# lixirui142/VidToMe

Hardware: AMD Instinct MI355X
Metric: denoising steps/sec, 16-frame 512x512 SD-1.5 chunk, ratio=0.5 (higher is better)
Workload: dtype f16 tokens; matching f16-MFMA filter + f32 exact refine (f32-identical indices); attention f16 MFMA with f32 accumulate

## Files before the change

### include/vidtome_hip.h

```cpp
#ifndef VIDTOME_HIP_H
#define VIDTOME_HIP_H

#include <stddef.h>
#include <stdint.h>

#ifdef __cplusplus
extern "C" {
#endif

#define VTM_ABI_VERSION 2

enum vtm_dtype { VTM_F32 = 0, VTM_F16 = 1, VTM_BF16 = 2 };

enum vtm_status {
    VTM_OK = 0,
    VTM_EINVAL = -1,
    VTM_ELAUNCH = -2,
    VTM_EWORKSPACE = -3
};

typedef void *vtm_stream_t;

int vtm_version(void);
const char *vtm_last_error(void);
// ... 128 lines not shown
                                    const int32_t *q_count, void *ws, size_t ws_bytes, vtm_stream_t stream);
size_t vtm_attention_kv_bounded_ws_bytes(int64_t B, int64_t h, int64_t Mq, int64_t Mk, int64_t d);

int vtm_transpose_cols(const void *x, int64_t ldx, int dtype, int64_t BF, int64_t N, int64_t C, void *out, int64_t ldo,
                       vtm_stream_t stream);

size_t vtm_fold_keys_ws_bytes(int64_t B, int64_t M, int64_t n_ids);
int vtm_fold_keys(const int32_t *cur, int64_t B, int64_t M, int64_t L, const int32_t *cid, int64_t Ma, int64_t n_ids,
                  int dtype, void *ws, size_t ws_bytes, int32_t *key_sel, uint32_t *k_bias, int64_t ldkb,
                  int32_t *k_count, vtm_stream_t stream);
int vtm_attention_kv_folded(const void *q, int64_t ldq, const void *k, int64_t ldk, const void *vt, int64_t ldvt,
                            void *out, int64_t ldo, int dtype, int64_t B, int64_t h, int64_t Mq, int64_t Mqp,
                            int64_t Mk, int64_t Mkp, int64_t d, float scale, const int32_t *q_count,
                            const int32_t *k_count, const uint32_t *k_bias, int64_t ldkb, void *ws, size_t ws_bytes,
                            vtm_stream_t stream);

size_t vtm_compact_queries_ws_bytes(int64_t B, int64_t Nd);
int vtm_compact_queries(const int32_t *loc, int64_t B, int64_t Ml, int64_t U, int64_t Nd, void *ws, size_t ws_bytes,
                        int32_t *qc, int32_t *tmap, int32_t *count, vtm_stream_t stream);

int64_t vtm_panel_rows(int64_t n);
int vtm_to_panels(const void *x, int dtype, int64_t rows, int64_t C, const int32_t *order, void *out, int64_t rows_pad,
                  vtm_stream_t stream);
int vtm_layernorm_panels(const void *x, const void *gamma, const void *beta, int dtype, int64_t rows, int64_t C, float eps,
                         void *out, int64_t panel_rows, vtm_stream_t stream);
int vtm_gather_panels(const void *x0, int64_t P0, const void *x1, int64_t P1, int dtype, int64_t B, int64_t C,
                      const int32_t *map, int64_t map_ld, const int32_t *map2, int64_t n, void *out, int64_t rows_per_sample,
                      vtm_stream_t stream);
int vtm_ff_geglu(const void *x_panels, int64_t n, int64_t n_pad, const void *w1_panels, int64_t D, int64_t w_rows_pad,
                 int64_t K, const float *bias, int dtype, void *out_panels, vtm_stream_t stream);
int vtm_linear_panels(const void *x_panels, int64_t n, int64_t n_pad, const void *w_panels, int64_t N, int64_t w_rows_pad,
                      int64_t K, const float *bias, const void *resid, int dtype, void *out, int64_t ldo,
                      vtm_stream_t stream);

int vtm_cfg_ddim(const void *x, const void *eps_uncond, const void *eps_cond, int dtype, int64_t n,
                 float guidance, float a, float b, float c, float d, void *eps_out, void *x_out,
                 vtm_stream_t stream);

int vtm_layernorm(const void *x, const void *gamma, const void *beta, int dtype, int64_t rows, int64_t C,
                  float eps, void *out, vtm_stream_t stream);

int vtm_geglu(const void *x, int dtype, int64_t rows, int64_t D, void *out, vtm_stream_t stream);

int vtm_linear_rows(const void *x0, int64_t P0, const void *x1, int64_t P1, int dtype, int64_t B, int64_t K,
                    const int32_t *rows, int64_t rows_ld, const int32_t *rows2, int64_t n, const void *W,
                    const void *bias, int64_t N, void *out, int64_t ldo, int64_t out_batch_stride,
                    int transposed, vtm_stream_t stream);

enum { VTM_LINEAR_NONE = 0, VTM_LINEAR_RESID = 1, VTM_LINEAR_GEGLU = 2 };
int vtm_linear_f32(const float *x0, int64_t P0, const float *x1, int64_t P1, int64_t B, int64_t K,
                   const int32_t *rows, int64_t rows_ld, const int32_t *rows2, int64_t n, const float *W,
                   const float *bias, int64_t N, int epilogue, const float *resid, void *out, int out_dtype,
                   int64_t ldo, int64_t out_batch_stride, int transposed, vtm_stream_t stream);

int vtm_lora_fold(const void *w, int dtype, const float *up, const float *down, int64_t c_out, int64_t c_in,
                  int64_t r, void *out, vtm_stream_t stream);

int vtm_dora_norms(const void *w, int dtype, const float *up, const float *down, int64_t c_out, int64_t c_in,
                   int64_t r, int64_t k_dora, float *norms, vtm_stream_t stream);
int vtm_dora_fold(const void *w, int dtype, const float *up, const float *down, const float *magnitude,
                  const float *norms, int64_t c_out, int64_t c_in, int64_t r, int64_t k_dora, void *out,
                  vtm_stream_t stream);

int vtm_loha_delta(const float *w1a, const float *w1b, const float *w2a, const float *w2b, int64_t c_out, int64_t c_in,
                   int64_t r, int accumulate, float *delta, vtm_stream_t stream);
int vtm_lokr_delta(const float *w1, const float *w2, int64_t a1, int64_t b1, int64_t a2, int64_t b2, int64_t c_out,
// ... 9 lines not shown
```

### vidtome_amd/_lib.py

```python
from __future__ import annotations

import ctypes
import functools
import os
import threading
from typing import Optional, Tuple

import torch

_HERE = os.path.dirname(os.path.abspath(__file__))
ABI_VERSION = 2
LIB_PATH = os.environ.get("VIDTOME_HIP_LIB") or os.path.join(_HERE, "lib", "libvidtome_hip.so")

VTM_F32, VTM_F16, VTM_BF16 = 0, 1, 2
ROW_PAD, K_PAD = 256, 32

_DT = {torch.float32: VTM_F32, torch.float16: VTM_F16, torch.bfloat16: VTM_BF16}

_vp, _i64, _int, _f32 = ctypes.c_void_p, ctypes.c_int64, ctypes.c_int, ctypes.c_float
_lib: Optional[ctypes.CDLL] = None

_SIGNATURES = {
    "vtm_version": ([], _int),
    "vtm_last_error": ([], ctypes.c_char_p),
# ... 29 lines not shown
    "vtm_unmerge_add": ([_vp, _i64, _vp, _vp, _int, _i64, _i64, _i64, _vp, _vp], _int),
    "vtm_merge_reduce": ([_vp, _int, _i64, _i64, _i64, _vp, _vp, _vp, _vp, _i64, _i64, _int, _vp, _i64, _i64, _vp], _int),
    "vtm_attention": ([_vp, _i64, _vp, _i64, _vp, _i64, _vp, _i64, _int, _i64, _i64, _i64, _i64, _i64, _f32,
                       _int, _vp, ctypes.c_size_t, _vp], _int),
    "vtm_attention_ws_bytes": ([_i64, _i64, _i64, _i64, _i64], ctypes.c_size_t),
    "vtm_attention_kv": ([_vp, _i64, _vp, _i64, _vp, _i64, _vp, _i64, _int, _i64, _i64, _i64, _i64, _i64, _i64, _i64,
                          _f32, _int, _vp, ctypes.c_size_t, _vp], _int),
    "vtm_attention_kv_sets": ([_vp, _i64, _vp, _i64, _vp, _i64, _vp, _i64, _int, _i64, _i64, _i64, _i64, _i64, _i64, _f32,
                               _int, ctypes.POINTER(_i64), ctypes.POINTER(_i64), ctypes.POINTER(_f32), _vp], _int),
    "vtm_attention_kv_sets_masked": ([_vp, _i64, _vp, _i64, _vp, _i64, _vp, _i64, _int, _i64, _i64, _i64, _i64, _i64, _i64, _f32,
                                      _int, ctypes.POINTER(_i64), ctypes.POINTER(_i64), ctypes.POINTER(_f32),
                                      ctypes.POINTER(_int), _vp, _i64, _i64, _vp], _int),
    "vtm_attention_kv_bias": ([_vp, _i64, _vp, _i64, _vp, _i64, _vp, _i64, _int, _i64, _i64, _i64, _i64, _i64, _i64, _i64,
                               _f32, _vp, _i64, _i64, _vp], _int),
    "vtm_attention_kv_bounded": ([_vp, _i64, _vp, _i64, _vp, _i64, _vp, _i64, _int, _i64, _i64, _i64, _i64, _i64, _i64, _i64,
                                  _f32, _vp, _vp, ctypes.c_size_t, _vp], _int),
    "vtm_attention_kv_shared_bounded": ([_vp, _i64, _vp, _i64, _vp, _i64, _vp, _i64, _int, _i64, _i64, _i64, _i64, _i64, _i64, _i64,
                                         _f32, _int, _vp, _vp, ctypes.c_size_t, _vp], _int),
    "vtm_attention_kv_bounded_ws_bytes": ([_i64, _i64, _i64, _i64, _i64], ctypes.c_size_t),
    "vtm_anchor_maps": ([_vp, _i64, _i64, _vp, _i64, _i64, _i64, _i64, _i64, _vp, _i64, _vp, _vp, _vp, _vp], _int),
    "vtm_transpose_cols": ([_vp, _i64, _int, _i64, _i64, _i64, _vp, _i64, _vp], _int),
    "vtm_fold_keys_ws_bytes": ([_i64, _i64, _i64], ctypes.c_size_t),
    "vtm_fold_keys": ([_vp, _i64, _i64, _i64, _vp, _i64, _i64, _int, _vp, ctypes.c_size_t, _vp, _vp, _i64, _vp, _vp], _int),
    "vtm_attention_kv_folded": ([_vp, _i64, _vp, _i64, _vp, _i64, _vp, _i64, _int, _i64, _i64, _i64, _i64, _i64, _i64, _i64,
                                 _f32, _vp, _vp, _vp, _i64, _vp, ctypes.c_size_t, _vp], _int),
    "vtm_compact_queries_ws_bytes": ([_i64, _i64], ctypes.c_size_t),
    "vtm_compact_queries": ([_vp, _i64, _i64, _i64, _i64, _vp, ctypes.c_size_t, _vp, _vp, _vp, _vp], _int),
    "vtm_panel_rows": ([_i64], _i64),
    "vtm_to_panels": ([_vp, _int, _i64, _i64, _vp, _vp, _i64, _vp], _int),
    "vtm_layernorm_panels": ([_vp, _vp, _vp, _int, _i64, _i64, _f32, _vp, _i64, _vp], _int),
    "vtm_gather_panels": ([_vp, _i64, _vp, _i64, _int, _i64, _i64, _vp, _i64, _vp, _i64, _vp, _i64, _vp], _int),
    "vtm_ff_geglu": ([_vp, _i64, _i64, _vp, _i64, _i64, _i64, _vp, _int, _vp, _vp], _int),
    "vtm_linear_panels": ([_vp, _i64, _i64, _vp, _i64, _i64, _i64, _vp, _vp, _int, _vp, _i64, _vp], _int),
    "vtm_cfg_ddim": ([_vp, _vp, _vp, _int, _i64, _f32, _f32, _f32, _f32, _f32, _vp, _vp, _vp], _int),
    "vtm_layernorm": ([_vp, _vp, _vp, _int, _i64, _i64, _f32, _vp, _vp], _int),
    "vtm_geglu": ([_vp, _int, _i64, _i64, _vp, _vp], _int),
    "vtm_linear_rows": ([_vp, _i64, _vp, _i64, _int, _i64, _i64, _vp, _i64, _vp, _i64, _vp, _vp, _i64, _vp, _i64, _i64,
                         _int, _vp], _int),
    "vtm_lora_fold": ([_vp, _int, _vp, _vp, _i64, _i64, _i64, _vp, _vp], _int),
    "vtm_dora_norms": ([_vp, _int, _vp, _vp, _i64, _i64, _i64, _i64, _vp, _vp], _int),
    "vtm_dora_fold": ([_vp, _int, _vp, _vp, _vp, _vp, _i64, _i64, _i64, _i64, _vp, _vp], _int),
    "vtm_loha_delta": ([_vp, _vp, _vp, _vp, _i64, _i64, _i64, _int, _vp, _vp], _int),
    "vtm_lokr_delta": ([_vp, _vp, _i64, _i64, _i64, _i64, _i64, _i64, _int, _vp, _vp], _int),
    "vtm_delta_fold": ([_vp, _int, _vp, _i64, _i64, _vp, _vp], _int),
    "vtm_linear_f32": ([_vp, _i64, _vp, _i64, _i64, _i64, _vp, _i64, _vp, _i64, _vp, _vp, _i64, _int, _vp, _vp, _int, _i64,
                        _i64, _int, _vp], _int),
}


def exported_symbols():
    return sorted(_SIGNATURES)


def lib() -> ctypes.CDLL:
    global _lib
    if _lib is None:
        if not os.path.exists(LIB_PATH):
            raise RuntimeError(
                f"{LIB_PATH} is missing: build it with `python -m vidtome_amd.build` (hipcc, gfx950). "
                "vidtome_amd has no CPU / eager fallback.")
        L = ctypes.CDLL(LIB_PATH)
        for name, (argtypes, restype) in _SIGNATURES.items():
            fn = getattr(L, name)
            fn.argtypes = argtypes
            fn.restype = restype
        if L.vtm_version() != ABI_VERSION:
# ... 719 lines not shown
    return out


@_on_device
def ff_geglu(x_panels: torch.Tensor, n: int, w1_panels: torch.Tensor, D: int, bias: Optional[torch.Tensor]) -> torch.Tensor:
    K = x_panels.shape[0] * 8
    out = torch.empty((D // 8, x_panels.shape[1], 8), dtype=x_panels.dtype, device=x_panels.device)
    _check(lib().vtm_ff_geglu(_ptr(x_panels), n, x_panels.shape[1], _ptr(w1_panels), D, w1_panels.shape[1], K, _ptr(bias),
                              dtype_code(x_panels), _ptr(out), _stream()), "vtm_ff_geglu")
    return out


@_on_device
def linear_panels(x_panels: torch.Tensor, n: int, w_panels: torch.Tensor, N: int, bias: Optional[torch.Tensor],
                  resid: Optional[torch.Tensor] = None, out: Optional[torch.Tensor] = None) -> torch.Tensor:
    K = x_panels.shape[0] * 8
    if x_panels.stride(2) != 1 or x_panels.stride(1) != 8 or w_panels.stride(2) != 1 or w_panels.stride(1) != 8 \
            or w_panels.shape[0] * 8 != K:
        raise RuntimeError("linear_panels: operands must be (K / 8, rows, 8) panel tensors (or row ranges of one)")
    if out is None:
        out = torch.empty((n, N), dtype=x_panels.dtype, device=x_panels.device)
    if out.stride(1) != 1 or out.shape[0] < n or out.shape[1] < N:
        raise RuntimeError("linear_panels: out must be an (n, N) view, contiguous along its rows")
    if resid is not None:
        _req(resid, "resid")
        if resid.numel() != n * N or resid.dtype != out.dtype or out.stride(0) != N:
            raise RuntimeError("linear_panels: residual shape / dtype mismatch")
    _check(lib().vtm_linear_panels(_ptr(x_panels), n, x_panels.stride(0) // 8, _ptr(w_panels), N, w_panels.stride(0) // 8, K,
                                   _ptr(bias), _ptr(resid), dtype_code(x_panels), out.data_ptr(), out.stride(0), _stream()),
           "vtm_linear_panels")
    return out


@_on_device
def gather_panels(x0: torch.Tensor, x1: Optional[torch.Tensor], rows: Optional[torch.Tensor], rows2: Optional[torch.Tensor],
                  n: int) -> torch.Tensor:
    _req(x0, "x0")
    B, P0, C = x0.shape
    P1 = 0 if x1 is None else _req(x1, "x1").shape[1]
    n_pad = panel_rows(n)
    out = torch.empty((C // 8, B * n_pad, 8), dtype=x0.dtype, device=x0.device)
    _check(lib().vtm_gather_panels(_ptr(x0), P0, _ptr(x1), P1, dtype_code(x0), B, C, _ptr(rows),
                                   0 if rows is None else rows.shape[1], _ptr(rows2), n, _ptr(out), n_pad, _stream()),
           "vtm_gather_panels")
    return out


@_on_device
def lora_fold(w: torch.Tensor, up: torch.Tensor, down: torch.Tensor, out: Optional[torch.Tensor] = None) -> torch.Tensor:
    _req(w, "w"), _req(up, "up"), _req(down, "down")
    c_out, c_in = w.shape
    r = up.shape[1]
    if up.dtype != torch.float32 or down.dtype != torch.float32 or tuple(up.shape) != (c_out, r) \
            or tuple(down.shape) != (r, c_in) or up.device != w.device or down.device != w.device:
        raise RuntimeError("lora_fold: up must be (c_out, r) and down (r, c_in) fp32 tensors on w's device")
    if out is None:
        out = torch.empty_like(w)
    _check(lib().vtm_lora_fold(_ptr(w), dtype_code(w), _ptr(up), _ptr(down), c_out, c_in, r, _ptr(_req(out, "out")),
                               _stream()), "vtm_lora_fold")
    return out


def _fold_operands(what: str, w: torch.Tensor, up: torch.Tensor, down: torch.Tensor, k_dora: int) -> Tuple[int, int, int]:
    _req(w, "w"), _req(up, "up"), _req(down, "down")
    c_out, c_in = w.shape
    r = up.shape[1]
# ... 96 lines not shown
```

### vidtome_amd/csrc/ff.hip

```cpp
#include "common.h"

#include <algorithm>
#include <cstdlib>
#include <type_traits>

namespace {

constexpr int FBD = 128;
constexpr int FBS = 256;
constexpr int FBK = 64;
constexpr int THREADS = 256;
constexpr int MAX_TILES_PER_WG = 16;

typedef float f32x16 __attribute__((ext_vector_type(16)));
typedef _Float16 h16x8 __attribute__((ext_vector_type(8)));
typedef __bf16 b16x8 __attribute__((ext_vector_type(8)));
typedef uint32_t u32x4 __attribute__((ext_vector_type(4)));
typedef __attribute__((address_space(3))) void lds_void;

template <typename T> struct Mma;
template <> struct Mma<__half> {
    __device__ static f32x16 run(u32x4 a, u32x4 b, f32x16 c) {
        return __builtin_amdgcn_mfma_f32_32x32x16_f16(__builtin_bit_cast(h16x8, a), __builtin_bit_cast(h16x8, b), c, 0, 0, 0);
    }
    __device__ static uint16_t bits(float v) { return __half_as_ushort(__float2half_rn(v)); }
    __device__ static float round(float v) { return __half2float(__float2half_rn(v)); }
};
template <> struct Mma<vtm_bf16> {
    __device__ static f32x16 run(u32x4 a, u32x4 b, f32x16 c) {
        return __builtin_amdgcn_mfma_f32_32x32x16_bf16(__builtin_bit_cast(b16x8, a), __builtin_bit_cast(b16x8, b), c, 0, 0, 0);
    }
    __device__ static uint16_t bits(float v) { return __bfloat16_as_ushort(__float2bfloat16(v)); }
    __device__ static float round(float v) { return __bfloat162float(__float2bfloat16(v)); }
};

__device__ __forceinline__ float gelu_erf(float g) {
    const float x = __builtin_fabsf(g) * 0.70710678118654752440f;
    const float t = __builtin_amdgcn_rcpf(__builtin_fmaf(0.3275911f, x, 1.0f));
    float p = __builtin_fmaf(1.061405429f, t, -1.453152027f);
    p = __builtin_fmaf(p, t, 1.421413741f);
    p = __builtin_fmaf(p, t, -0.284496736f);
    p = __builtin_fmaf(p, t, 0.254829592f);
    const float e = p * t * __builtin_amdgcn_exp2f(-x * x * 1.4426950408889634f);
    return 0.5f * g * (g < 0.0f ? e : 2.0f - e);
}

enum { EPI_GEGLU = 0, EPI_ROWS = 1 };

struct Epi {
    const float *bias;
    void *out;
    int64_t out_rows_pad;
    int64_t ldo;
    const void *resid;
    int64_t n;
    int64_t N;
    int64_t nbias;
};

template <typename T, int EPI>
__global__ __launch_bounds__(THREADS, 2) void panel_gemm_kernel(
    const uint4 *__restrict__ ah, const uint4 *__restrict__ bh, int64_t Ns_pad, int64_t Nd_pad, int64_t C_pad,
    int ns_tiles, int nd_tiles, int nsplit, int tiles_per_split, int total_src_tiles, int patch_tiles, Epi E) {
    __shared__ __attribute__((aligned(16))) uint4 sA[2][8 * FBD];
    __shared__ float sBias[MAX_TILES_PER_WG * FBD];
    __shared__ __attribute__((aligned(16))) uint16_t sOut[EPI == EPI_ROWS ? 4 * 32 * (FBD + 8) : 8];

    const int tid = threadIdx.x, lane = tid & 63;
    const int wave = __builtin_amdgcn_readfirstlane(tid >> 6);
    const int l31 = lane & 31, kh = lane >> 5;

    const int xcd = blockIdx.x & 7, slot = blockIdx.x >> 3;
    const int per_group = patch_tiles * nsplit;
    const int grp = (slot / per_group) * 8 + xcd;
    const int q = slot % per_group;
    const int stg = grp * patch_tiles + q % patch_tiles;
    const int split = q / patch_tiles;
    if (stg >= total_src_tiles) return;
    const int st_ = stg % ns_tiles;
    const int jt0 = split * tiles_per_split;
    const int jt1 = min(jt0 + tiles_per_split, nd_tiles);
    if (jt0 >= jt1) return;

    const int KT = (int)(C_pad / FBK);
    const int steps = (jt1 - jt0) * KT;
    const uint4 *srch = ah, *dsth = bh;
    const int64_t srow0 = (int64_t)st_ * FBS + wave * 64;

    __shared__ Epi sE;
    if (tid == 0) sE = E;
    {
        const int cnt = (jt1 - jt0) * FBD;
        const float *bsrc = E.bias != nullptr ? E.bias + (int64_t)jt0 * FBD : nullptr;
#pragma unroll
        for (int k = 0; k < MAX_TILES_PER_WG * FBD / THREADS; ++k) {
            const int i = tid + k * THREADS;
            if (i < cnt) sBias[i] = (bsrc != nullptr && (int64_t)jt0 * FBD + i < E.nbias) ? bsrc[i] : 0.0f;
        }
    }

    constexpr int NB = 2, PG = 2;
    const uint32_t voff_b = (uint32_t)(kh * Ns_pad + srow0 + l31) * 16u;
    const int64_t bgroup = 2 * Ns_pad;
    u32x4 rb[4][2];
    auto await_b = [&](auto count_tag, u32x4 (&r)[2]) {
// ... 147 lines not shown
                    if constexpr (s < 3) fn[j] = __builtin_bit_cast(u32x4, sA[buf][((s + 1) * 2 + kh) * FBD + j * 32 + l31]);
                    else fn[j] = __builtin_bit_cast(u32x4, sA[buf ^ 1][kh * FBD + j * 32 + l31]);
                } else if (j < 6) {
                    if constexpr (s < 2) load_b1(pb, s + 2, j - 4, rb[s + 2][j - 4]);
                    else load_b1(pbn, s - 2, j - 4, rb[s - 2][j - 4]);
                } else {
                    if constexpr (s == 0) load_a_piece(pa1, buf ^ 1, j - 4);
                    if constexpr (s == 3) load_a_piece(pa2, buf, j - 6);
                    if constexpr (s == 1)
                        asm volatile("global_load_dword %0, %1, %2" : "=v"(am[j - 6]) : "v"(voff_m), "s"(dummy_rows));
                }
                __builtin_amdgcn_sched_barrier(0);
            }
        };
        await_b(std::integral_constant<int, NB + PG>{}, rb[0]);
        if (kt == 0) group(std::integral_constant<int, 0>{}, std::true_type{});
        else group(std::integral_constant<int, 0>{}, std::false_type{});
        group(std::integral_constant<int, 1>{}, std::false_type{});
        group(std::integral_constant<int, 2>{}, std::false_type{});
        asm volatile("s_waitcnt vmcnt(%0) lgkmcnt(0)" ::"n"(2 * NB + 2) : "memory");
        __syncthreads();
        group(std::integral_constant<int, 3>{}, std::false_type{});
        if (wrap) {
            epilogue(jt);
            ++jt;
        }
        kt = kt1;
        pb = pbn;
        pa1 = pa2;
    }
    asm volatile("s_waitcnt vmcnt(0)" ::: "memory");
}

template <typename T>
__global__ __launch_bounds__(256) void to_panels_kernel(const T *__restrict__ x, int64_t rows, int64_t C, int64_t rows_pad,
                                                        const int32_t *__restrict__ order, uint4 *__restrict__ out) {
    const int64_t G = C / 8;
    const int64_t i = (int64_t)blockIdx.x * blockDim.x + threadIdx.x;
    if (i >= rows_pad * G) return;
    const int64_t g = i % G, r = i / G;
    uint4 v = make_uint4(0, 0, 0, 0);
    if (r < rows) {
        const int64_t src = order ? order[r] : r;
        if (src >= 0) v = *reinterpret_cast<const uint4 *>(x + src * C + g * 8);
    }
    out[g * rows_pad + r] = v;
}

template <typename T>
__global__ __launch_bounds__(256) void gather_panels_kernel(const T *__restrict__ x0, int64_t P0, const T *__restrict__ x1,
                                                            int64_t P1, int64_t B, int64_t C, const int32_t *__restrict__ map,
                                                            int64_t map_ld, const int32_t *__restrict__ map2, int64_t n,
                                                            int64_t rows_per_sample, int64_t stride, uint4 *__restrict__ out) {
    const int64_t G = C / 8;
    const int64_t i = (int64_t)blockIdx.x * blockDim.x + threadIdx.x;
    if (i >= B * rows_per_sample * G) return;
    const int64_t g = i % G, r = (i / G) % rows_per_sample, b = i / (G * rows_per_sample);
    uint4 v = make_uint4(0, 0, 0, 0);
    if (r < n) {
        int64_t p = map2 ? map2[b * n + r] : r;
        if (map) p = map[b * map_ld + p];
        const T *row = p < P0 ? x0 + (b * P0 + p) * C : x1 + (b * P1 + (p - P0)) * C;
        v = *reinterpret_cast<const uint4 *>(row + g * 8);
    }
    out[g * stride + b * rows_per_sample + r] = v;
}
// ... 40 lines not shown
                       (const __half *)x, rows, C, rows_pad, order, (uint4 *)out);
    return vtm::launch_status("vtm_to_panels");
}

VTM_EXPORT int vtm_gather_panels(const void *x0, int64_t P0, const void *x1, int64_t P1, int dtype, int64_t B, int64_t C,
                                 const int32_t *map, int64_t map_ld, const int32_t *map2, int64_t n, void *out,
                                 int64_t rows_per_sample, vtm_stream_t stream) {
    VTM_REQUIRE(x0 && out && B > 0 && C > 0 && C % 8 == 0 && n > 0, "vtm_gather_panels: bad arguments");
    VTM_REQUIRE(P1 == 0 || x1, "vtm_gather_panels: x1 is null but P1 > 0");
    VTM_REQUIRE(map || map2 || n <= P0 + P1, "vtm_gather_panels: identity rows must lie inside the pool");
    VTM_REQUIRE(!map || map_ld > 0, "vtm_gather_panels: map_ld");
    VTM_REQUIRE(rows_per_sample >= n && rows_per_sample % FBS == 0, "vtm_gather_panels: rows_per_sample must be a multiple of 256 >= n");
    VTM_REQUIRE(dtype == VTM_F16 || dtype == VTM_BF16, "vtm_gather_panels: dtype must be VTM_F16 or VTM_BF16");
    const int64_t total = B * rows_per_sample * (C / 8);
    hipLaunchKernelGGL(gather_panels_kernel<__half>, dim3((unsigned)vtm::cdiv(total, 256)), dim3(256), 0, vtm::as_stream(stream),
                       (const __half *)x0, P0, (const __half *)x1, P1, B, C, map, map_ld, map2, n, rows_per_sample,
                       B * rows_per_sample, (uint4 *)out);
    return vtm::launch_status("vtm_gather_panels");
}

VTM_EXPORT int vtm_ff_geglu(const void *x_panels, int64_t n, int64_t n_pad, const void *w1_panels, int64_t D, int64_t w_rows_pad,
                            int64_t K, const float *bias, int dtype, void *out_panels, vtm_stream_t stream) {
    VTM_REQUIRE(x_panels && w1_panels && out_panels, "vtm_ff_geglu: null pointer");
    VTM_REQUIRE(n > 0 && n_pad >= n && n_pad % FBS == 0, "vtm_ff_geglu: token rows must be padded to 256");
    VTM_REQUIRE(D > 0 && D % 64 == 0 && w_rows_pad >= 2 * D && w_rows_pad % FBS == 0, "vtm_ff_geglu: D %% 64, packed weight rows padded to 256");
    VTM_REQUIRE(K > 0 && K % FBK == 0, "vtm_ff_geglu: K must be a multiple of 64");
    Epi E{bias, out_panels, n_pad, 0, nullptr, n, D, 2 * D};
    hipStream_t s = vtm::as_stream(stream);
    if (dtype == VTM_F16) return launch_panel_gemm<__half, EPI_GEGLU>(x_panels, n, n_pad, w1_panels, 2 * D, w_rows_pad, K, E, s);
    if (dtype == VTM_BF16) return launch_panel_gemm<vtm_bf16, EPI_GEGLU>(x_panels, n, n_pad, w1_panels, 2 * D, w_rows_pad, K, E, s);
    return vtm::fail(VTM_EINVAL, "vtm_ff_geglu: dtype must be VTM_F16 or VTM_BF16");
}

VTM_EXPORT int vtm_linear_panels(const void *x_panels, int64_t n, int64_t n_pad, const void *w_panels, int64_t N, int64_t w_rows_pad,
                                 int64_t K, const float *bias, const void *resid, int dtype, void *out, int64_t ldo,
                                 vtm_stream_t stream) {
    VTM_REQUIRE(x_panels && w_panels && out, "vtm_linear_panels: null pointer");
    VTM_REQUIRE(n > 0 && n_pad >= vtm::cdiv(n, FBS) * FBS, "vtm_linear_panels: token rows must be padded to 256");
    VTM_REQUIRE(N > 0 && N % 8 == 0 && w_rows_pad >= vtm::cdiv(N, FBD) * FBD, "vtm_linear_panels: N %% 8, weight rows padded to 128");
    VTM_REQUIRE(K > 0 && K % FBK == 0, "vtm_linear_panels: K must be a multiple of 64");
    VTM_REQUIRE(ldo >= N && ldo % 8 == 0 && (reinterpret_cast<uintptr_t>(out) & 15) == 0 &&
                    (reinterpret_cast<uintptr_t>(resid) & 15) == 0, "vtm_linear_panels: output rows must be 16-byte aligned");
    Epi E{bias, out, 0, ldo, resid, n, N, N};
    hipStream_t s = vtm::as_stream(stream);
    if (dtype == VTM_F16) return launch_panel_gemm<__half, EPI_ROWS>(x_panels, n, n_pad, w_panels, N, w_rows_pad, K, E, s);
    if (dtype == VTM_BF16) return launch_panel_gemm<vtm_bf16, EPI_ROWS>(x_panels, n, n_pad, w_panels, N, w_rows_pad, K, E, s);
    return vtm::fail(VTM_EINVAL, "vtm_linear_panels: dtype must be VTM_F16 or VTM_BF16");
}
```

### vidtome_amd/patch.py

```python
from __future__ import annotations

import math
import os
from typing import Any, Callable, Dict, Optional, Tuple, Type

import torch
import torch.nn.functional as F

from . import _lib, ip_adapter, lora, merge
from .utils import init_generator, isinstance_str, join_frame, split_frame

LIVE_QUERIES = os.environ.get("VIDTOME_LIVE_QUERIES", "1") != "0"
COMPACT_QUERIES = os.environ.get("VIDTOME_COMPACT_QUERIES", "1") != "0"


class MergePlan:

    __slots__ = ("fsize", "L", "M", "gather_map", "_inv", "_inv_parts", "_merged", "levels", "global_level", "local_chunk",
                 "x_joined", "anchors_in", "q_rows", "inv_q", "q_count", "pad_to", "fold_args", "_key_fold", "aligned")

    def __init__(self):
        self.levels = []
        self.global_level = None
        self.local_chunk = None
# ... 323 lines not shown
    to_out = attn.to_out
    return to_out[0] if isinstance(to_out, (torch.nn.ModuleList, torch.nn.Sequential, list, tuple)) else to_out


def fused_attention_ok(attn: torch.nn.Module, x: torch.Tensor, self_attn: bool = True,
                       processors=_PLAIN_PROCESSORS) -> bool:
    if not (x.is_cuda and x.dim() == 3 and x.dtype in (torch.float16, torch.bfloat16, torch.float32)):
        return False
    if not all(hasattr(attn, a) for a in ("to_q", "to_k", "to_v", "to_out", "heads")):
        return False
    if not all(_readable_linear(m) for m in (attn.to_q, attn.to_k, attn.to_v, _out_linear(attn))):
        return False
    C = x.shape[-1]
    if lora.base_linear(attn.to_q).out_features != C or C % attn.heads or (C // attn.heads) not in _HEAD_DIMS:
        return False
    if any(getattr(attn, a, None) is not None for a in ("group_norm", "spatial_norm", "norm_cross", "norm_q", "norm_k")):
        return False
    if getattr(attn, "rescale_output_factor", 1.0) != 1.0 or getattr(attn, "residual_connection", False):
        return False
    proc = getattr(attn, "processor", None)
    if proc is not None and type(proc).__name__ not in processors:
        return False
    if "forward" in attn.__dict__ and not (self_attn and _pnp_num_inputs(attn) is not None):
        return False
    to_out = attn.to_out
    if attn.training and isinstance(to_out, (torch.nn.ModuleList, torch.nn.Sequential)) and len(to_out) > 1 \
            and getattr(to_out[1], "p", 0.0) != 0.0:
        return False
    return True


PROJ_MODE = os.environ.get("VIDTOME_PROJ", "auto")
FUSED_PROJ = PROJ_MODE != "blas"


def _proj_dtypes_ok(attn: torch.nn.Module, dtype) -> bool:
    for lin in (attn.to_q, attn.to_k, attn.to_v, _out_linear(attn)):
        if not _linear_dtype_ok(lin, dtype):
            return False
    return True


def _linear_dtype_ok(lin: torch.nn.Module, dtype) -> bool:
    base = lora.base_linear(lin)
    return base.weight.dtype == dtype and (base.bias is None or base.bias.dtype == dtype)


def _has_bias(lin: torch.nn.Module) -> bool:
    return lora.linear_params(lin)[1] is not None


def fused_projections_ok(attn: torch.nn.Module, x: torch.Tensor) -> bool:
    if not FUSED_PROJ or x.dtype not in (torch.float16, torch.bfloat16) or x.shape[-1] % 32 \
            or not _proj_dtypes_ok(attn, x.dtype):
        return False
    return PROJ_MODE == "rows" or (PROJ_MODE == "auto" and x.shape[-1] <= 320)


def panel_projections_ok(attn: torch.nn.Module, x: torch.Tensor) -> bool:
    return (PROJ_MODE in ("auto", "panels") and x.dtype in (torch.float16, torch.bfloat16) and x.shape[-1] % 64 == 0
            and _proj_dtypes_ok(attn, x.dtype) and not _has_bias(attn.to_v))


def _panel_weight(lin: torch.nn.Module):
    w, b, key = _linear(lin)
    return _packed(lin, "rows", key, w.device, lambda: (_lib.to_panels(w.detach().contiguous()),
                                                       None if b is None else b.detach().float().contiguous()))


def self_attention_panels(attn: torch.nn.Module, x0: torch.Tensor, x1: Optional[torch.Tensor], rows: Optional[torch.Tensor],
                          q_rows: Optional[torch.Tensor] = None, q_count: Optional[torch.Tensor] = None) -> torch.Tensor:
    B, _, C = x0.shape
    M = x0.shape[1] if rows is None else rows.shape[1]
    heads = attn.heads
    scale = getattr(attn, "scale", None) or (C // heads) ** -0.5
    share = _pnp_share_groups(attn)
    Mpad = _lib.panel_rows(M)
    xp = _lib.gather_panels(x0, x1, rows, None, M)
    wq, bq = _panel_weight(attn.to_q)
    wk, bk = _panel_weight(attn.to_k)
    wv, _ = _panel_weight(attn.to_v)
    k_op = _lib.linear_panels(xp, B * Mpad, wk, C, bk).view(B, Mpad, C)
    vt = torch.empty((B, C, Mpad), dtype=x0.dtype, device=x0.device)
    M8 = (M + 7) // 8 * 8
    for b in range(B):
        _lib.linear_panels(wv, C, xp[:, b * Mpad:(b + 1) * Mpad], M8, None, out=vt[b])
    if q_rows is None:
        q_op = _lib.linear_panels(xp, B * Mpad, wq, C, bq).view(B, Mpad, C)
        o = _lib.attention(q_op, k_op, vt, heads, M, scale, share)
        Mq, Mqpad = M, Mpad
    else:
        Mq = q_rows.shape[1]
        Mqpad = _lib.panel_rows(Mq)
        qp = _lib.gather_panels(x0, x1, rows, q_rows, Mq)
        q_op = _lib.linear_panels(qp, B * Mqpad, wq, C, bq).view(B, Mqpad, C)
        o = _lib.attention_kv(q_op, k_op, vt, heads, Mq, M, scale, q_count=q_count, share_groups=share)
    wo, bo = _panel_weight(_out_linear(attn))
    op = _lib.to_panels(o.view(B * Mqpad, C))
    return _lib.linear_panels(op, B * Mqpad, wo, C, bo).view(B, Mqpad, C)


def unmerged_site(block: torch.nn.Module, x: torch.Tensor) -> bool:
    info = block._tome_info
    if info["size"] is None:
        return False
    downsample = int(math.ceil(math.sqrt((info["size"][0] * info["size"][1]) // x.shape[1])))
    return downsample > info["args"]["max_downsample"]


def unmerged_self_attention_ok(block: torch.nn.Module, x: torch.Tensor) -> bool:
    norm, attn = block.norm1, block.attn1
    return (x.is_cuda and x.dim() == 3 and type(norm) is torch.nn.LayerNorm and len(norm.normalized_shape) == 1
            and norm.normalized_shape[0] == x.shape[-1] and (norm.weight is None or norm.weight.dtype == x.dtype)
            and (norm.bias is None or norm.bias.dtype == x.dtype) and fused_attention_ok(attn, x)
            and panel_projections_ok(attn, x) and not fused_projections_ok(attn, x) and _pnp_share_groups(attn) == 1
            and unmerged_site(block, x))


def unmerged_self_attention_residual(block: torch.nn.Module, hidden_states: torch.Tensor) -> torch.Tensor:
    attn, norm = block.attn1, block.norm1
    BF, N, C = hidden_states.shape
    heads = attn.heads
    scale = getattr(attn, "scale", None) or (C // heads) ** -0.5
    hs = hidden_states.contiguous()
    n = BF * N

    qkv_params = [_linear(m) for m in (attn.to_q, attn.to_k, attn.to_v)]

# ... 133 lines not shown
    if q_rows is None:
        qk = F.linear(x, wqk, bqk).to(core)
        q_op, k_op = qk[:, :, :C], qk[:, :, C:]
    else:
        xq = _lib.gather_rows(x, None, q_rows, pad_to=8)
        q_op = F.linear(xq, wqk[:C], None if bqk is None else bqk[:C]).to(core)
        k_op = F.linear(x, wqk[C:], None if bqk is None else bqk[C:]).to(core)
    wv, bv, _ = _linear(attn.to_v, x.dtype)
    if B <= 4:
        vt = torch.empty((B, C, Mp), dtype=x.dtype, device=x.device)
        for bi in range(B):
            torch.mm(wv, x[bi].t(), out=vt[bi])
    else:
        vt = torch.matmul(wv, x.transpose(1, 2))
    if bv is not None:
        vt = vt + bv[None, :, None]
    vt = vt.to(core)
    if q_rows is None:
        o = _lib.attention(q_op, k_op, vt, heads, M, scale, share)
    else:
        o = _lib.attention_kv(q_op, k_op, vt, heads, q_rows.shape[1], M, scale, q_count=q_count, share_groups=share)
    o = o.to(x.dtype)
    wo, bo, _ = _linear(_out_linear(attn), o.dtype)
    return F.linear(o, wo, bo)


def _cross_kv(to_k: torch.nn.Module, to_v: torch.nn.Module, enc: torch.Tensor, C: int, panels: bool = True):
    B, Mkp, D = enc.shape
    dt = enc.dtype
    if panels and D % 64 == 0 and lora.base_linear(to_k).weight.dtype == dt and lora.base_linear(to_v).weight.dtype == dt:
        ep = _lib.to_panels(enc.reshape(B * Mkp, D))
        wk, bk = _panel_weight(to_k)
        wv, bv = _panel_weight(to_v)
        k = _lib.linear_panels(ep, B * Mkp, wk, C, bk).view(B, Mkp, C)
        vt = _lib.linear_panels(ep, B * Mkp, wv, C, bv).view(B, Mkp, C).transpose(1, 2).contiguous()
    else:
        if panels:
            _warn_once("lib-cross-kv", f"vidtome_amd: attn2's k / v projections run as library GEMMs (conditioning width "
                                       f"{D} is not a multiple of 64, or to_k / to_v are not of the tokens' dtype)")
        k = _apply_linear(to_k, enc)
        vt = _apply_linear(to_v, enc).transpose(1, 2).contiguous()
    return k, vt


def _pad_keys(enc: torch.Tensor, dt) -> torch.Tensor:
    enc = enc.to(dt)
    pad = -enc.shape[1] % 8
    return F.pad(enc, (0, 0, 0, pad)) if pad else enc


def _ip_key_sets(attn: torch.nn.Module, ip: "ip_adapter.Call", dt, C: int, panels: bool):
    lens = [im.shape[1] for im in ip.images]
    masks = ip.masks if ip.masks is not None else [None] * len(lens)
    images = [0 if m is None else m.shape[0] for m in masks]
    if any(images):
        sets, active, _, rows = ip_adapter.masked_key_sets(ip.text.shape[1], lens, ip.scales, images)
    else:
        (sets, active, _), rows = ip_adapter.key_sets(ip.text.shape[1], lens, ip.scales), []
    k, vt = _cross_kv(attn.to_k, attn.to_v, _pad_keys(ip.text, dt), C, panels)
    if active:
        parts = [(k, vt)]
        for a in active:
            ka, vta = _cross_kv(ip.k_proj[a], ip.v_proj[a], _pad_keys(ip.images[a], dt), C, panels)
            t = lens[a] // max(images[a], 1)
            if images[a] > 1 and t % 8:
                pad = -t % 8
                ka = torch.cat([F.pad(ka[:, i * t:(i + 1) * t], (0, 0, 0, pad)) for i in range(images[a])], dim=1)
                vta = torch.cat([F.pad(vta[:, :, i * t:(i + 1) * t], (0, pad)) for i in range(images[a])], dim=2)
# ... 512 lines not shown
```

Measured before the change: 22.05.

## Batch Q/K/V panel projections into one grouped GEMM launch

Adds a grouped panel-GEMM kernel that takes up to eight independent projection problems in a single launch. Each workgroup finds its problem from block-offset tables, and a planner picks a shared tiles-per-workgroup target to balance the combined grid across CUs. Self-attention K, per-sample V-transpose and Q projections, plus cross-attention K/V, now go through it by default. The aim is to cut launch overhead and fill the idle CUs left by small individual GEMMs, at the cost of a different split heuristic and a larger kernel-argument struct.

```diff
diff --git a/include/vidtome_hip.h b/include/vidtome_hip.h
--- a/include/vidtome_hip.h
+++ b/include/vidtome_hip.h
@@ -184,6 +184,17 @@
 int vtm_linear_panels(const void *x_panels, int64_t n, int64_t n_pad, const void *w_panels, int64_t N, int64_t w_rows_pad,
                       int64_t K, const float *bias, const void *resid, int dtype, void *out, int64_t ldo,
                       vtm_stream_t stream);
+typedef struct vtm_panel_problem {
+    const void *x_panels;
+    int64_t n, n_pad;
+    const void *w_panels;
+    int64_t N, w_rows_pad, K;
+    const float *bias;
+    const void *resid;
+    void *out;
+    int64_t ldo;
+} vtm_panel_problem;
+int vtm_linear_panels_grouped(const vtm_panel_problem *problems, int count, int dtype, vtm_stream_t stream);
 
 int vtm_cfg_ddim(const void *x, const void *eps_uncond, const void *eps_cond, int dtype, int64_t n,
                  float guidance, float a, float b, float c, float d, void *eps_out, void *x_out,
diff --git a/vidtome_amd/_lib.py b/vidtome_amd/_lib.py
--- a/vidtome_amd/_lib.py
+++ b/vidtome_amd/_lib.py
@@ -85,6 +85,7 @@
     "vtm_gather_panels": ([_vp, _i64, _vp, _i64, _int, _i64, _i64, _vp, _i64, _vp, _i64, _vp, _i64, _vp], _int),
     "vtm_ff_geglu": ([_vp, _i64, _i64, _vp, _i64, _i64, _i64, _vp, _int, _vp, _vp], _int),
     "vtm_linear_panels": ([_vp, _i64, _i64, _vp, _i64, _i64, _i64, _vp, _vp, _int, _vp, _i64, _vp], _int),
+    "vtm_linear_panels_grouped": ([_vp, _int, _int, _vp], _int),
     "vtm_cfg_ddim": ([_vp, _vp, _vp, _int, _i64, _f32, _f32, _f32, _f32, _f32, _vp, _vp, _vp], _int),
     "vtm_layernorm": ([_vp, _vp, _vp, _int, _i64, _i64, _f32, _vp, _vp], _int),
     "vtm_geglu": ([_vp, _int, _i64, _i64, _vp, _vp], _int),
@@ -870,6 +871,44 @@
     return out
 
 
+class _PanelProblem(ctypes.Structure):
+    _fields_ = [("x_panels", _vp), ("n", _i64), ("n_pad", _i64), ("w_panels", _vp), ("N", _i64), ("w_rows_pad", _i64),
+                ("K", _i64), ("bias", _vp), ("resid", _vp), ("out", _vp), ("ldo", _i64)]
+
+
+MAX_PANEL_PROBLEMS = 8
+
+
+def linear_panels_grouped(problems) -> list:
+    if not 1 <= len(problems) <= MAX_PANEL_PROBLEMS:
+        raise RuntimeError("linear_panels_grouped: 1 to 8 problems")
+    return _linear_panels_grouped(problems[0][0].device, problems)
+
+
+@_on_device
+def _linear_panels_grouped(device: torch.device, problems) -> list:
+    dt = problems[0][0].dtype
+    arr = (_PanelProblem * len(problems))()
+    outs = []
+    for i, (x_panels, n, w_panels, N, bias, out) in enumerate(problems):
+        K = x_panels.shape[0] * 8
+        if x_panels.stride(2) != 1 or x_panels.stride(1) != 8 or w_panels.stride(2) != 1 or w_panels.stride(1) != 8 \
+                or w_panels.shape[0] * 8 != K:
+            raise RuntimeError("linear_panels_grouped: operands must be (K / 8, rows, 8) panel tensors (or row ranges of one)")
+        if x_panels.dtype != dt or w_panels.dtype != dt or x_panels.device != device:
+            raise RuntimeError("linear_panels_grouped: one dtype and one device per call")
+        if out is None:
+            out = torch.empty((n, N), dtype=dt, device=x_panels.device)
+        if out.stride(1) != 1 or out.shape[0] < n or out.shape[1] < N or out.dtype != dt:
+            raise RuntimeError("linear_panels_grouped: out must be an (n, N) view, contiguous along its rows")
+        arr[i] = _PanelProblem(_ptr(x_panels), n, x_panels.stride(0) // 8, _ptr(w_panels), N, w_panels.stride(0) // 8, K,
+                               _ptr(bias), None, out.data_ptr(), out.stride(0))
+        outs.append(out)
+    _check(lib().vtm_linear_panels_grouped(ctypes.addressof(arr), len(problems), dtype_code(problems[0][0]), _stream()),
+           "vtm_linear_panels_grouped")
+    return outs
+
+
 @_on_device
 def gather_panels(x0: torch.Tensor, x1: Optional[torch.Tensor], rows: Optional[torch.Tensor], rows2: Optional[torch.Tensor],
                   n: int) -> torch.Tensor:
diff --git a/vidtome_amd/csrc/ff.hip b/vidtome_amd/csrc/ff.hip
--- a/vidtome_amd/csrc/ff.hip
+++ b/vidtome_amd/csrc/ff.hip
@@ -1,4 +1,5 @@
 #include "common.h"
+#include "panel_plan.h"
 
 #include <algorithm>
 #include <cstdlib>
@@ -11,6 +12,8 @@
 constexpr int FBK = 64;
 constexpr int THREADS = 256;
 constexpr int MAX_TILES_PER_WG = 16;
+static_assert(FBD == vtm_panel_plan::FBD && FBS == vtm_panel_plan::FBS && FBK == vtm_panel_plan::FBK &&
+              MAX_TILES_PER_WG == vtm_panel_plan::MAX_TILES_PER_WG, "panel_plan.h plans for these tiles");
 
 typedef float f32x16 __attribute__((ext_vector_type(16)));
 typedef _Float16 h16x8 __attribute__((ext_vector_type(8)));
@@ -59,9 +62,10 @@
 };
 
 template <typename T, int EPI>
-__global__ __launch_bounds__(THREADS, 2) void panel_gemm_kernel(
+__device__ __forceinline__ void panel_gemm_body(
     const uint4 *__restrict__ ah, const uint4 *__restrict__ bh, int64_t Ns_pad, int64_t Nd_pad, int64_t C_pad,
-    int ns_tiles, int nd_tiles, int nsplit, int tiles_per_split, int total_src_tiles, int patch_tiles, Epi E) {
+    int ns_tiles, int nd_tiles, int nsplit, int tiles_per_split, int total_src_tiles, int patch_tiles, const Epi &E,
+    int block) {
     __shared__ __attribute__((aligned(16))) uint4 sA[2][8 * FBD];
     __shared__ float sBias[MAX_TILES_PER_WG * FBD];
     __shared__ __attribute__((aligned(16))) uint16_t sOut[EPI == EPI_ROWS ? 4 * 32 * (FBD + 8) : 8];
@@ -70,7 +74,7 @@
     const int wave = __builtin_amdgcn_readfirstlane(tid >> 6);
     const int l31 = lane & 31, kh = lane >> 5;
 
-    const int xcd = blockIdx.x & 7, slot = blockIdx.x >> 3;
+    const int xcd = block & 7, slot = block >> 3;
     const int per_group = patch_tiles * nsplit;
     const int grp = (slot / per_group) * 8 + xcd;
     const int q = slot % per_group;
@@ -284,6 +288,38 @@
     asm volatile("s_waitcnt vmcnt(0)" ::: "memory");
 }
 
+template <typename T, int EPI>
+__global__ __launch_bounds__(THREADS, 2) void panel_gemm_kernel(
+    const uint4 *__restrict__ ah, const uint4 *__restrict__ bh, int64_t Ns_pad, int64_t Nd_pad, int64_t C_pad,
+    int ns_tiles, int nd_tiles, int nsplit, int tiles_per_split, int total_src_tiles, int patch_tiles, Epi E) {
+    panel_gemm_body<T, EPI>(ah, bh, Ns_pad, Nd_pad, C_pad, ns_tiles, nd_tiles, nsplit, tiles_per_split, total_src_tiles,
+                            patch_tiles, E, (int)blockIdx.x);
+}
+
+struct GroupProblem {
+    const uint4 *tok, *w;
+    int64_t tok_pad, w_pad, K;
+    int ns_tiles, nd_tiles, nsplit, tiles_per_split, total_src_tiles, patch_tiles;
+    int first;
+    Epi E;
+};
+struct GroupArgs {
+    int count;
+    GroupProblem p[vtm_panel_plan::MAX_PROBLEMS];
+};
+
+template <typename T>
+__global__ __launch_bounds__(THREADS, 2) void panel_gemm_grouped_kernel(const GroupArgs G) {
+    const int blk = (int)blockIdx.x;
+    int pi = 0;
+#pragma unroll
+    for (int i = 1; i < vtm_panel_plan::MAX_PROBLEMS; ++i)
+        if (i < G.count && blk >= G.p[i].first) pi = i;
+    const GroupProblem &P = G.p[pi];
+    panel_gemm_body<T, EPI_ROWS>(P.tok, P.w, P.tok_pad, P.w_pad, P.K, P.ns_tiles, P.nd_tiles, P.nsplit, P.tiles_per_split,
+                                 P.total_src_tiles, P.patch_tiles, P.E, blk - P.first);
+}
+
 template <typename T>
 __global__ __launch_bounds__(256) void to_panels_kernel(const T *__restrict__ x, int64_t rows, int64_t C, int64_t rows_pad,
                                                         const int32_t *__restrict__ order, uint4 *__restrict__ out) {
@@ -390,15 +426,58 @@
     return vtm::fail(VTM_EINVAL, "vtm_ff_geglu: dtype must be VTM_F16 or VTM_BF16");
 }
 
-VTM_EXPORT int vtm_linear_panels(const void *x_panels, int64_t n, int64_t n_pad, const void *w_panels, int64_t N, int64_t w_rows_pad,
-                                 int64_t K, const float *bias, const void *resid, int dtype, void *out, int64_t ldo,
-                                 vtm_stream_t stream) {
+namespace {
+
+int check_linear_panels(const void *x_panels, int64_t n, int64_t n_pad, const void *w_panels, int64_t N, int64_t w_rows_pad,
+                        int64_t K, const void *resid, const void *out, int64_t ldo) {
     VTM_REQUIRE(x_panels && w_panels && out, "vtm_linear_panels: null pointer");
     VTM_REQUIRE(n > 0 && n_pad >= vtm::cdiv(n, FBS) * FBS, "vtm_linear_panels: token rows must be padded to 256");
     VTM_REQUIRE(N > 0 && N % 8 == 0 && w_rows_pad >= vtm::cdiv(N, FBD) * FBD, "vtm_linear_panels: N %% 8, weight rows padded to 128");
     VTM_REQUIRE(K > 0 && K % FBK == 0, "vtm_linear_panels: K must be a multiple of 64");
     VTM_REQUIRE(ldo >= N && ldo % 8 == 0 && (reinterpret_cast<uintptr_t>(out) & 15) == 0 &&
                     (reinterpret_cast<uintptr_t>(resid) & 15) == 0, "vtm_linear_panels: output rows must be 16-byte aligned");
+    return VTM_OK;
+}
+
+template <typename T>
+int launch_panel_group(const vtm_panel_problem *pr, int count, hipStream_t s) {
+    namespace pp = vtm_panel_plan;
+    pp::Problem shapes[pp::MAX_PROBLEMS];
+    for (int i = 0; i < count; ++i) shapes[i] = pp::Problem{pr[i].n, pr[i].N, pr[i].K};
+    const pp::GroupPlan P = pp::plan_group(shapes, count, vtm::device_cus(), pp::debug_tiles_target());
+    if (P.grid >= (1ll << 31)) return vtm::fail(VTM_EINVAL, "vtm_linear_panels_grouped: grid too large");
+    GroupArgs G{};
+    G.count = count;
+    for (int i = 0; i < count; ++i) {
+        const pp::Geometry &g = P.g[i];
+        G.p[i] = GroupProblem{(const uint4 *)pr[i].x_panels, (const uint4 *)pr[i].w_panels, pr[i].n_pad, pr[i].w_rows_pad, pr[i].K,
+                              g.ns_tiles, g.nd_tiles, g.nsplit, g.tiles_per_split, g.total_src_tiles, g.patch_tiles,
+                              (int)P.first[i],
+                              Epi{pr[i].bias, pr[i].out, 0, pr[i].ldo, pr[i].resid, pr[i].n, pr[i].N, pr[i].N}};
+    }
+    hipLaunchKernelGGL((panel_gemm_grouped_kernel<T>), dim3((unsigned)P.grid), dim3(THREADS), 0, s, G);
+    return vtm::launch_status("vtm_linear_panels_grouped");
+}
+
+}
+
+VTM_EXPORT int vtm_linear_panels_grouped(const vtm_panel_problem *problems, int count, int dtype, vtm_stream_t stream) {
+    VTM_REQUIRE(problems && count >= 1 && count <= vtm_panel_plan::MAX_PROBLEMS, "vtm_linear_panels_grouped: 1 to 8 problems");
+    VTM_REQUIRE(dtype == VTM_F16 || dtype == VTM_BF16, "vtm_linear_panels_grouped: dtype must be VTM_F16 or VTM_BF16");
+    for (int i = 0; i < count; ++i) {
+        const vtm_panel_problem &p = problems[i];
+        if (int rc = check_linear_panels(p.x_panels, p.n, p.n_pad, p.w_panels, p.N, p.w_rows_pad, p.K, p.resid, p.out, p.ldo)) return rc;
+        VTM_REQUIRE(2 * p.n_pad * 16 < (1ll << 32), "panel GEMM: %lld token panel rows exceed the 32-bit fragment offset",
+                    (long long)p.n_pad);
+    }
+    hipStream_t s = vtm::as_stream(stream);
+    return dtype == VTM_F16 ? launch_panel_group<__half>(problems, count, s) : launch_panel_group<vtm_bf16>(problems, count, s);
+}
+
+VTM_EXPORT int vtm_linear_panels(const void *x_panels, int64_t n, int64_t n_pad, const void *w_panels, int64_t N, int64_t w_rows_pad,
+                                 int64_t K, const float *bias, const void *resid, int dtype, void *out, int64_t ldo,
+                                 vtm_stream_t stream) {
+    if (int rc = check_linear_panels(x_panels, n, n_pad, w_panels, N, w_rows_pad, K, resid, out, ldo)) return rc;
     Epi E{bias, out, 0, ldo, resid, n, N, N};
     hipStream_t s = vtm::as_stream(stream);
     if (dtype == VTM_F16) return launch_panel_gemm<__half, EPI_ROWS>(x_panels, n, n_pad, w_panels, N, w_rows_pad, K, E, s);
diff --git a/vidtome_amd/csrc/panel_plan.h b/vidtome_amd/csrc/panel_plan.h
--- /dev/null
+++ b/vidtome_amd/csrc/panel_plan.h
@@ -0,0 +1,113 @@
+#pragma once
+#include <cstdint>
+#include <cstdlib>
+
+namespace vtm_panel_plan {
+
+constexpr int FBD = 128;
+constexpr int FBS = 256;
+constexpr int FBK = 64;
+constexpr int MAX_TILES_PER_WG = 16;
+constexpr int MAX_PROBLEMS = 8;
+
+inline int64_t cdiv(int64_t a, int64_t b) { return (a + b - 1) / b; }
+
+struct Problem {
+    int64_t n, Nw, K;
+};
+
+struct Geometry {
+    int ns_tiles, nd_tiles, total_src_tiles, patch_tiles, ngroups;
+    int nsplit, tiles_per_split;
+    int64_t grid;
+};
+
+inline void patch_geometry(Geometry &G, int64_t n, int64_t Nw, int64_t K) {
+    G.ns_tiles = (int)cdiv(n, FBS);
+    G.nd_tiles = (int)cdiv(Nw, FBD);
+    G.total_src_tiles = G.ns_tiles;
+    const int max_patch = (int64_t)16 * FBS * K * 2 <= (3 << 20) ? 16 : 8;
+    const int tiles_per_xcd = (int)cdiv(G.total_src_tiles, 8);
+    const int patches_per_xcd = (int)cdiv(tiles_per_xcd, max_patch);
+    G.patch_tiles = (int)cdiv(tiles_per_xcd, patches_per_xcd);
+    G.ngroups = (int)cdiv(G.total_src_tiles, G.patch_tiles);
+}
+
+inline void set_splits(Geometry &G, int64_t nsplit) {
+    const int64_t lo = cdiv(G.nd_tiles, MAX_TILES_PER_WG);
+    nsplit = nsplit < lo ? lo : nsplit;
+    nsplit = nsplit < 1 ? 1 : nsplit > G.nd_tiles ? G.nd_tiles : nsplit;
+    G.tiles_per_split = (int)cdiv(G.nd_tiles, nsplit);
+    G.nsplit = (int)cdiv(G.nd_tiles, G.tiles_per_split);
+    G.grid = (int64_t)8 * cdiv(G.ngroups, 8) * G.patch_tiles * G.nsplit;
+}
+
+inline Geometry plan_single(int64_t n, int64_t Nw, int64_t K, int cus) {
+    Geometry G;
+    patch_geometry(G, n, Nw, K);
+    const int64_t slots = (int64_t)cus * 2;
+    set_splits(G, cdiv(3 * slots, (int64_t)G.ns_tiles));
+    return G;
+}
+
+struct GroupPlan {
+    int count;
+    Geometry g[MAX_PROBLEMS];
+    int64_t first[MAX_PROBLEMS];
+    int64_t grid;
+    int tiles_target;
+};
+
+inline int debug_tiles_target() {
+    static const int t = [] {
+        const char *v = getenv("VTM_DEBUG_PANEL_TPS");
+        return v ? atoi(v) : -1;
+    }();
+    return t;
+}
+
+inline int64_t active_wgs(const Geometry &G, int t) {
+    Geometry H = G;
+    set_splits(H, cdiv(G.nd_tiles, t));
+    return (int64_t)H.ns_tiles * H.nsplit;
+}
+
+inline int choose_tiles_target(const Geometry *g, int count, int cus) {
+    const int64_t slots = (int64_t)cus * 2;
+    int max_nd = 1;
+    for (int i = 0; i < count; ++i) max_nd = g[i].nd_tiles > max_nd ? g[i].nd_tiles : max_nd;
+    double best_cost = 1e30;
+    int best = 1;
+    for (int t = 1; t <= MAX_TILES_PER_WG && t <= max_nd; ++t) {
+        int64_t wgs = 0;
+        for (int i = 0; i < count; ++i) wgs += active_wgs(g[i], t);
+        if (t > 1 && wgs < slots) break;
+        int64_t rounds = cdiv(wgs, slots);
+        const int64_t last = wgs - (rounds - 1) * slots;
+        if (last > slots - slots / 16) ++rounds;
+        const double cost = (double)rounds * (t + 1.5);
+        if (cost < best_cost - 1e-9) {
+            best_cost = cost;
+            best = t;
+        }
+    }
+    return best;
+}
+
+inline GroupPlan plan_group(const Problem *p, int count, int cus, int forced_t = -1) {
+    GroupPlan P;
+    P.count = count;
+    for (int i = 0; i < count; ++i) patch_geometry(P.g[i], p[i].n, p[i].Nw, p[i].K);
+    const int t = forced_t > 0 ? (forced_t > MAX_TILES_PER_WG ? MAX_TILES_PER_WG : forced_t) : choose_tiles_target(P.g, count, cus);
+    P.tiles_target = t;
+    int64_t at = 0;
+    for (int i = 0; i < count; ++i) {
+        set_splits(P.g[i], cdiv(P.g[i].nd_tiles, t));
+        P.first[i] = at;
+        at = cdiv(at + P.g[i].grid, 8) * 8;
+    }
+    P.grid = at;
+    return P;
+}
+
+}
diff --git a/vidtome_amd/patch.py b/vidtome_amd/patch.py
--- a/vidtome_amd/patch.py
+++ b/vidtome_amd/patch.py
@@ -379,6 +379,7 @@
 
 PROJ_MODE = os.environ.get("VIDTOME_PROJ", "auto")
 FUSED_PROJ = PROJ_MODE != "blas"
+GROUPED_PANELS = os.environ.get("VIDTOME_GROUPED_PANELS", "1") != "0"
 
 
 def _proj_dtypes_ok(attn: torch.nn.Module, dtype) -> bool:
@@ -427,20 +428,25 @@
     wq, bq = _panel_weight(attn.to_q)
     wk, bk = _panel_weight(attn.to_k)
     wv, _ = _panel_weight(attn.to_v)
-    k_op = _lib.linear_panels(xp, B * Mpad, wk, C, bk).view(B, Mpad, C)
     vt = torch.empty((B, C, Mpad), dtype=x0.dtype, device=x0.device)
     M8 = (M + 7) // 8 * 8
-    for b in range(B):
-        _lib.linear_panels(wv, C, xp[:, b * Mpad:(b + 1) * Mpad], M8, None, out=vt[b])
     if q_rows is None:
-        q_op = _lib.linear_panels(xp, B * Mpad, wq, C, bq).view(B, Mpad, C)
-        o = _lib.attention(q_op, k_op, vt, heads, M, scale, share)
-        Mq, Mqpad = M, Mpad
+        Mq, Mqpad, qp = M, Mpad, xp
     else:
         Mq = q_rows.shape[1]
         Mqpad = _lib.panel_rows(Mq)
         qp = _lib.gather_panels(x0, x1, rows, q_rows, Mq)
-        q_op = _lib.linear_panels(qp, B * Mqpad, wq, C, bq).view(B, Mqpad, C)
+    probs = [(xp, B * Mpad, wk, C, bk, None)]
+    probs += [(wv, C, xp[:, b * Mpad:(b + 1) * Mpad], M8, None, vt[b]) for b in range(B)]
+    probs.append((qp, B * Mqpad, wq, C, bq, None))
+    if GROUPED_PANELS and len(probs) <= _lib.MAX_PANEL_PROBLEMS:
+        outs = _lib.linear_panels_grouped(probs)
+    else:
+        outs = [_lib.linear_panels(x, n, w, N, bias, out=out) for x, n, w, N, bias, out in probs]
+    k_op, q_op = outs[0].view(B, Mpad, C), outs[-1].view(B, Mqpad, C)
+    if q_rows is None:
+        o = _lib.attention(q_op, k_op, vt, heads, M, scale, share)
+    else:
         o = _lib.attention_kv(q_op, k_op, vt, heads, Mq, M, scale, q_count=q_count, share_groups=share)
     wo, bo = _panel_weight(_out_linear(attn))
     op = _lib.to_panels(o.view(B * Mqpad, C))
@@ -640,8 +646,12 @@
         ep = _lib.to_panels(enc.reshape(B * Mkp, D))
         wk, bk = _panel_weight(to_k)
         wv, bv = _panel_weight(to_v)
-        k = _lib.linear_panels(ep, B * Mkp, wk, C, bk).view(B, Mkp, C)
-        vt = _lib.linear_panels(ep, B * Mkp, wv, C, bv).view(B, Mkp, C).transpose(1, 2).contiguous()
+        if GROUPED_PANELS:
+            k, v = _lib.linear_panels_grouped([(ep, B * Mkp, wk, C, bk, None), (ep, B * Mkp, wv, C, bv, None)])
+        else:
+            k, v = _lib.linear_panels(ep, B * Mkp, wk, C, bk), _lib.linear_panels(ep, B * Mkp, wv, C, bv)
+        k = k.view(B, Mkp, C)
+        vt = v.view(B, Mkp, C).transpose(1, 2).contiguous()
     else:
         if panels:
             _warn_once("lib-cross-kv", f"vidtome_amd: attn2's k / v projections run as library GEMMs (conditioning width "
```

After: 22.25, median of 4. Within noise of the previous version (+0.9%).
